# laoreja/HPLFlowNet

Hardware: AMD Instinct MI355X
Metric: point-pairs/sec + EPE3D, N=8192 FlyingThings3D, 1/2/4/8 MI355X (higher is better)
Workload: dtype f32 (wide layers: fp32 operands as scaled fp16 pairs, 3 partial products, fp32 accumulate); 1 GPU; full HPLFlowNet inference (7 levels, 19.3M params, random init), FT3D-like synthetic pair, N=8192, bs=1 per GPU; num_points=8192, step_includes_lattice_build=True, forward_streams=3, lattices_under_construction=3, exact_fallback_launches=0, lattice_launches_per_pair=34

## Files before the change

hplflownet_amd/bcl.py:

```python
import collections

import os

import torch
import torch.nn as nn

from . import _lib, ops
from .ops import ACT_LEAKY, ACT_NONE, LEAKY_RATE

__all__ = ['BilateralConvFlex', 'BilateralCorrelationFlex', 'sparse_sum', 'Conv1dReLU', 'Conv2dReLU',
           'Conv3dReLU', 'LEAKY_RATE']


class _ConvReLU(nn.Module):
    conv_cls = None

    def __init__(self, in_channels, out_channels, kernel_size=1, stride=1, padding=0, use_leaky=False,
                 bias=True):
        super(_ConvReLU, self).__init__()
        self.in_channels, self.out_channels, self.kernel_size = in_channels, out_channels, kernel_size
        self.use_leaky = use_leaky
        relu = nn.LeakyReLU(LEAKY_RATE, inplace=True) if use_leaky else nn.ReLU(inplace=True)
        self.composed_module = nn.Sequential(
            self.conv_cls(in_channels, out_channels, kernel_size=kernel_size, stride=stride, padding=padding,
# ... 215 lines not shown
        return ops.splat_raw(v, (csr_ptr, csr_pt, csr_w, norm), H, use_norm=False)

    @staticmethod
    def backward(ctx, grad_output):
        indices, = ctx.saved_tensors
        g = None
        if ctx.needs_input_grad[1]:
            g = grad_output[indices.reshape(-1).to(grad_output.device), :]
        return None, g, None, None


sparse_sum = SparseSum.apply


def _build_conv_stack(n_in, num_output, filter_size, last_relu, use_leaky, first_cls=Conv2dReLU,
                      plain_cls=nn.Conv2d):
    mods = []
    c = n_in
    for i, o in enumerate(num_output):
        ks = (filter_size, 1) if i == 0 else (1, 1)
        last = i == len(num_output) - 1
        if last and not last_relu:
            mods.append(plain_cls(c, o, kernel_size=ks))
        else:
            mods.append(first_cls(c, o, ks, use_leaky=use_leaky))
        c = o
    return nn.Sequential(*mods)


def _conv_of(m):
    return m.conv if isinstance(m, _ConvReLU) else m


def _run_conv_stack(x, stack, table, M, F, use_leaky, out=None, w0=None):
    n = len(stack)
    for i, m in enumerate(stack):
        conv = _conv_of(m)
        act = ACT_LEAKY if isinstance(m, _ConvReLU) else ACT_NONE
        o = out if i == n - 1 else None
        if i == 0:
            groups = table.groups() if conv.in_channels >= GROUPS_MIN_CHANNELS else None
            x = ops.gconv(x, conv.weight if w0 is None else w0, conv.bias, table.t, M, F, act=act,
                          bwd_mode=table.bwd_mode(x.shape[0]) if torch.is_grad_enabled() else 'scatter',
                          out=o, slope=_slope(use_leaky),
                          row_perm=table.perm if groups is None else None,
                          taps=table.taps if conv.in_channels >= 100 else None, tap_groups=groups,
                          reg_stride=getattr(table, 'reg_stride', 0),
                          tiles=(table.group_tiles() if groups is not None else table.perm_tiles) if table.t is not None else None)
        else:
            x = ops.gconv(x, conv.weight, conv.bias, None, M, 1, act=act, bwd_mode='dense', out=o,
                          slope=_slope(use_leaky))
    return x


class BilateralConvFlex(nn.Module):

    def __init__(self, d, neighborhood_size, num_input, num_output, DEVICE, use_bias, use_leaky, use_norm,
                 do_splat, do_slice, last_relu, chunk_size=1024 * 1024 * 25):
        super(BilateralConvFlex, self).__init__()
        self.d, self.d1 = d, d + 1
        self.neighborhood_size = neighborhood_size
        self.filter_size = (neighborhood_size + 1) ** self.d1 - neighborhood_size ** self.d1
        self.num_input, self.num_output = num_input, list(num_output)
        self.DEVICE = DEVICE
        self.use_bias, self.use_leaky, self.use_norm = use_bias, use_leaky, use_norm
        self.do_splat, self.do_slice, self.last_relu = do_splat, do_slice, last_relu
        self.MAX_SIZE = chunk_size
        self.register_buffer('feat_indices', torch.arange(num_input, dtype=torch.long))
        if do_slice:
            self.register_buffer('out_indices', torch.arange(num_output[-1], dtype=torch.long))
        self.blur_conv = _build_conv_stack(num_input, self.num_output, self.filter_size, last_relu, use_leaky)
        if do_slice and use_bias:
            self.register_parameter('bias', nn.Parameter(torch.zeros((num_output[-1],), dtype=torch.float32)))

    def get_filter_size(self):
        return self.filter_size

    def forward_cl(self, x, in_cloud, blur, out_cloud, out=None, keep=None, w0=None, folded=False):
        H = blur.t.shape[1]
        if self.do_splat:
            if in_cloud.H != H:
# ... 3 lines not shown
            else:
                s = ops.splat_raw(x, in_cloud.csr(), H, self.use_norm)
        else:
            if x.shape[0] != H:
                raise _lib.HplError('features have %d rows, blur table %d vertices' % (x.shape[0], H))
            s = x
        bias = (self.bias if self.use_bias else None) if self.do_slice else None
        mods = list(self.blur_conv)
        if folded:
            if torch.is_grad_enabled() or not self.do_slice or len(mods) < 2 or isinstance(mods[-1], _ConvReLU):
                raise _lib.HplError('the folded form is the inference forward of a slicing layer that ends in a bias-only 1x1')
            y = _run_conv_stack(s, mods[:-1], blur, H, self.filter_size, self.use_leaky, w0=w0)
            if keep is not None:
                keep.append(y)
            return ops.slice_raw(y, out_cloud.bary, out_cloud.off, out_cloud.N, out=out)
        if (self.do_slice and len(mods) >= 2 and not isinstance(mods[-1], _ConvReLU) and out_cloud.N < H):
            y = _run_conv_stack(s, mods[:-1], blur, H, self.filter_size, self.use_leaky)
            if keep is not None:
                keep.append(y)
            conv = mods[-1]
            b = conv.bias if bias is None else (conv.bias + bias if conv.bias is not None else bias)
            if torch.is_grad_enabled() and y.requires_grad:
                z = ops.SliceFn.apply(y, out_cloud, None)
            else:
                z = ops.slice_raw(y, out_cloud.bary, out_cloud.off, out_cloud.N)
            return ops.gconv(z, conv.weight, b, None, out_cloud.N, 1, act=ACT_NONE, bwd_mode='dense', out=out)
        if keep is not None and self.do_slice and len(mods) >= 2 and not isinstance(mods[-1], _ConvReLU):
            z = _run_conv_stack(s, mods[:-1], blur, H, self.filter_size, self.use_leaky)
            keep.append(z)
            conv = _conv_of(mods[-1])
            y = ops.gconv(z, conv.weight, conv.bias, None, H, 1, act=ACT_NONE, bwd_mode='dense', slope=_slope(self.use_leaky))
        else:
            y = _run_conv_stack(s, self.blur_conv, blur, H, self.filter_size, self.use_leaky,
                                out=None if self.do_slice else out)
            if keep is not None:
                keep.append(y)
        if not self.do_slice:
            return y
        if torch.is_grad_enabled() and (y.requires_grad or (bias is not None and bias.requires_grad)):
            z = ops.SliceFn.apply(y, out_cloud, bias)
            if out is not None:
                out.copy_(z)
                return out
            return z
        return ops.slice_raw(y, out_cloud.bary, out_cloud.off, out_cloud.N, bias=bias, out=out)

    def forward(self, features, in_barycentric, in_lattice_offset, blur_neighbors, out_barycentric,
                out_lattice_offset):
        if features.size(0) != 1:
            raise _lib.HplError('batch size must be 1 (reference README.md:57)')
        x = to_channel_last(features)
        H = blur_neighbors.size(-1)
        blur = nbr_table(blur_neighbors, x)
        in_cloud = cloud_tables(in_barycentric, in_lattice_offset, H, x) if self.do_splat else None
        out_cloud = cloud_tables(out_barycentric, out_lattice_offset, H, x) if self.do_slice else None
        return to_channel_first(self.forward_cl(x, in_cloud, blur, out_cloud))


class BilateralCorrelationFlex(nn.Module):

    def __init__(self, d, corr_filter_radius, corr_corr_radius, num_input, num_corr_output, num_output, DEVICE,
                 use_bias, use_leaky, use_norm, prev_corr_dim, last_relu, chunk_size=1024 * 1024 * 25):
        super(BilateralCorrelationFlex, self).__init__()
        self.d, self.d1 = d, d + 1
        self.corr_size = (corr_corr_radius + 1) ** self.d1 - corr_corr_radius ** self.d1
        self.filter_size = (corr_filter_radius + 1) ** self.d1 - corr_filter_radius ** self.d1
        self.num_input, self.prev_corr_dim = num_input, prev_corr_dim
# ... 68 lines not shown
```

hplflownet_amd/build.py:

```python
import os
import subprocess
import sys

HERE = os.path.dirname(os.path.abspath(__file__))
CSRC = os.path.join(HERE, 'csrc')
LIB = os.path.join(HERE, 'libhplbcl.so')
DIAG_LIB = os.path.join(HERE, 'libhplbcl_diag.so')
SOURCES = ['index_ops.hip', 'row_order.hip', 'splat_slice.hip', 'train_ops.hip', 'gconv.hip', 'gconv3.hip', 'wgrad3.hip', 'lattice.hip', 'lattice_fused.hip', 'executor.hip', 'lattice_builder.hip', 'lattice_query.hip', 'knn_interp.hip', 'rigid_fit.hip', 'motion_segment.hip', 'selfsup_loss.hip', 'ground_fit.hip', 'batch_io.hip', 'metrics.hip', 'transforms.hip']
FLAGS = ['--offload-arch=gfx950', '-O3', '-std=c++17', '-fPIC', '-munsafe-fp-atomics',
         '-ffp-contract=off',
         '-Wall', '-Wno-unused-function']


def needs_build():
    if not os.path.exists(LIB) or not os.path.exists(DIAG_LIB):
        return True
    t = os.path.getmtime(LIB)
    deps = [os.path.join(CSRC, f) for f in os.listdir(CSRC)] + \
           [os.path.join(os.path.dirname(HERE), 'include', 'hpl_bcl.h'), os.path.abspath(__file__)]
    return any(os.path.getmtime(d) > t for d in deps)


def build(force=False, verbose=False):
    if not force and not needs_build():
        return LIB
    hipcc = os.environ.get('HIPCC', '/opt/rocm/bin/hipcc')
    objs = []
    procs = []
    for src in SOURCES:
        path = os.path.join(CSRC, src)
        if not os.path.exists(path):
            continue
        obj = os.path.join(CSRC, src.replace('.hip', '.o'))
        cmd = [hipcc] + FLAGS + ['-c', path, '-o', obj]
        if verbose:
            print(' '.join(cmd))
        procs.append((src, subprocess.Popen(cmd, stdout=subprocess.PIPE, stderr=subprocess.STDOUT)))
        objs.append(obj)
    failed = False
    for src, p in procs:
        out, _ = p.communicate()
# ... 13 lines not shown
```

hplflownet_amd/csrc/gconv.hip:

```cpp
#include "common.h"
#include "gconv_common.h"
#include <cstdlib>
#include <cmath>
#include <string>

#include <stdlib.h>
#include <type_traits>

using namespace hpl;
using namespace hpl_gc;



namespace {

template <int BM, int BN, int WGM, int WGN, bool AVEC, int F_LDS, bool COMPACT = false>
__global__ void __launch_bounds__(64 * WGM * WGN, COMPACT ? 6 : 1) k_gconv(const GParams p) {
    constexpr int NT = 64 * WGM * WGN;
    constexpr int WTM = BM / WGM, WTN = BN / WGN;
    constexpr int TM = WTM / 32, TN = WTN / 32;
    constexpr int LDA_S = COMPACT ? BM + 1 : BM + 2;
    constexpr int LDB_S = BN;
    constexpr int A_ROWS_PER_PASS = NT / 8;
    constexpr int A_PASSES = BM / A_ROWS_PER_PASS;
// ... 582 lines not shown
    if (p.F == 1) {
        if (avec) k_gconv<BM, BN, WGM, WGN, true, 1><<<grid, 64 * WGM * WGN, 0, s>>>(p);
        else k_gconv<BM, BN, WGM, WGN, false, 1><<<grid, 64 * WGM * WGN, 0, s>>>(p);
    } else {
        if (avec) k_gconv<BM, BN, WGM, WGN, true, 15><<<grid, 64 * WGM * WGN, 0, s>>>(p);
        else k_gconv<BM, BN, WGM, WGN, false, 15><<<grid, 64 * WGM * WGN, 0, s>>>(p);
    }
}

}

namespace {
void launch_finish(const GParams &p, hipStream_t s) {
    const bool vec = p.N % 4 == 0 && p.ldy % 4 == 0 && aligned16(p.Y) && aligned16(p.partial) && (!p.bias || aligned16(p.bias)) &&
                     (!p.res || (p.ldres % 4 == 0 && aligned16(p.res))) && (!p.Y2 || (p.ldy2 % 4 == 0 && aligned16(p.Y2))) &&
                     p.M * p.N < (int64_t)0x7fffffff && p.res_mod < (int64_t)0x7fffffff;
    if (vec) {
        const int g = (int)imin(cdiv(p.M * (p.N / 4), 256), 2048);
        k_gconv_finish4<<<g, 256, 0, s>>>(p);
    } else {
        const int g = (int)imin(cdiv(p.M * p.N, 256), 2048);
        k_gconv_finish<<<g, 256, 0, s>>>(p);
    }
}
}

extern "C" int hpl_gconv_forward(const hpl_gconv_desc *d, hplStream stream) {
    GParams p;
    int rc = fill_params(d, p, "hpl_gconv_forward");
    if (rc != HPL_OK) return rc;
    if (p.M == 0) return HPL_OK;
    hipStream_t s = to_stream(stream);
    const bool avec = (p.C % 4 == 0) && (p.lda % 4 == 0) && aligned16(p.A);
    if (avec && p.Wt3 && launch_split3(p, s)) {
        if (p.splits > 1) launch_finish(p, s);
        HPL_CHECK_LAUNCH("hpl_gconv_forward");
        if (p.y_amax && !p.y_amax_done) return amax_launch(p.Y, p.ldy, p.M, p.N, p.y_amax, s, p.y_guard);
        return HPL_OK;
    }
    const int64_t t128 = cdiv(p.M, 128), t64 = cdiv(p.M, 64);
    const int nsel = p.N;
    if (nsel > 64) {
        const int64_t tn = cdiv(p.N, 128);
        if (t64 * tn >= 512) launch_cfg<64, 128, 2, 4>(p, avec, s);
        else launch_cfg<64, 64, 2, 2>(p, avec, s);
    } else if (nsel > 32) {
        launch_cfg<64, 64, 2, 2>(p, avec, s);
    } else {
        if (t128 >= 512) launch_cfg<128, 32, 4, 1>(p, avec, s);
        else launch_cfg<64, 32, 2, 1>(p, avec, s);
    }
    if (p.splits > 1) launch_finish(p, s);
    HPL_CHECK_LAUNCH("hpl_gconv_forward");
    if (p.y_amax) return amax_launch(p.Y, p.ldy, p.M, p.N, p.y_amax, s, p.y_guard);
    return HPL_OK;
}

namespace {
__global__ void __launch_bounds__(256) k_tile_index(const int32_t *__restrict__ nbr, int64_t stride, int F, int64_t M,
                                                    const int32_t *__restrict__ perm, int BM, int32_t *__restrict__ tile_idx,
                                                    int32_t *__restrict__ tile_mask) {
    __shared__ int masks[8];
    const int t = threadIdx.x;
    if (t < 8) masks[t] = 0;
    __syncthreads();
    const int64_t tile = blockIdx.x, m0 = tile * BM;
// ... 736 lines not shown
```

hplflownet_amd/csrc/gconv_common.h:

```cpp
#pragma once
#include "common.h"

namespace hpl_gc {

typedef float floatx16 __attribute__((ext_vector_type(16)));
typedef int int32x4_t __attribute__((ext_vector_type(4)));
typedef float float4_t __attribute__((ext_vector_type(4)));

__device__ float4_t buffer_load_f32x4(int32x4_t srsrc, int voffset, int soffset, int aux)
    __asm("llvm.amdgcn.raw.buffer.load.v4f32");


__device__ __forceinline__ int32x4_t make_rsrc(const void *base, int bytes) {
    union {
        int32x4_t v;
        struct { const void *p; int range; int cfg; } s;
    } u;
    u.s.p = base;
    u.s.range = bytes;
    u.s.cfg = 0x00020000;
    return u.v;
}

__host__ __device__ __forceinline__ float split_scale(float amax) {
// ... 94 lines not shown
        for (; x < 8; ++x) {
            int rows_x = 0;
            for (int r = 0; r * 8 < nchunks; ++r) {
                const int c = chunk_of(x, r);
                if (c < nchunks) rows_x += chunk_rows(c);
            }
            if (sq < rows_x) break;
            sq -= rows_x;
        }
        int row = 0;
        for (int r = 0;; ++r) {
            const int c = chunk_of(x, r);
            if (c >= nchunks) continue;
            const int n = chunk_rows(c);
            if (sq < n) { row = c * G + sq; break; }
            sq -= n;
        }
        tm = T - 1 - row;
        return;
    }
    constexpr int BAND = 8;
    const int band_sz = BAND * p.tiles_n;
    const int band = id / band_sz;
    const int in_band = id - band * band_sz;
    const int rows_in_band = min(BAND, p.tiles_m - band * BAND);
    tm = band * BAND + in_band % rows_in_band;
    tn = in_band / rows_in_band;
}
__device__ __forceinline__ void tile_coords(const GParams &p, int &tm, int &tn) { tile_coords(p, tm, tn, blockIdx.x); }


int fill_params(const hpl_gconv_desc *d, GParams &p, const char *who);
bool launch_split3(GParams &p, hipStream_t s);
bool split3_enabled();
int split_planes();
int amax_launch(const float *X, int64_t ld, int64_t rows, int cols, float *slot, hipStream_t s, unsigned *guard = nullptr);
constexpr int GUARD_GAP = 18;
__device__ __forceinline__ bool guard_tripped(const float *a_amax, const unsigned *a_guard) {
    if (!a_guard || !a_amax) return false;
    unsigned am;
    const float amf = a_amax[0];
    __builtin_memcpy(&am, &amf, 4);
    const unsigned g = a_guard[0];
    const unsigned rmin = g ? ~g : am;
    return (am >> 23) >= (rmin >> 23) + (unsigned)GUARD_GAP && (am >> 23) < 255u;
}
constexpr int RESID_SHIFT = 24;
inline bool split3_maybe(int64_t M, int C, int F, int N) {
    if (!(C >= 32 && N >= 256 && M >= 1024 && F <= 15)) return false;
    const int64_t tiles256 = ((M + 127) / 128) * ((N + 255) / 256);
    if (tiles256 >= 128) return true;
    if (F == 1) return M >= 8192;
    if (M >= 16384) return true;
    const int64_t nk = ((int64_t)F * C + BK - 1) / BK;
    const int64_t by_tiles = 256 / tiles256, by_k = nk / 16;
    return N % 256 == 0 && (by_tiles < by_k ? by_tiles : by_k) >= 2;
}

struct WParams {
    const float *A; int64_t lda; const int32_t *nbr; int64_t nbr_stride; int64_t reg_stride;
    int64_t M; int C; int F; int K;
    const float *dY; int64_t lddy; int N;
    float *dWt; int64_t ldw;
    int tiles_n; int64_t m_per_split;
    const int32_t *tap_m; const int32_t *tap_row; const int32_t *tap_ptr; int c_tiles;
    float *dbias;
// ... 7 lines not shown
```

hplflownet_amd/ops.py:

```python
import collections
import ctypes
import os

import torch

from . import _lib
from ._lib import GConvDesc, RelayoutJob, check, ptr, stream

ACT_NONE, ACT_LEAKY = 0, 1
LEAKY_RATE = 0.1


def _cl(x, what='activation'):
    if x.dim() != 2 or x.dtype != torch.float32 or not x.is_cuda or (x.shape[1] > 1 and x.stride(1) != 1):
        raise _lib.HplError('%s must be a channel-last 2-D float32 device tensor with unit channel stride, '
                            'got shape %s strides %s dtype %s device %s'
                            % (what, tuple(x.shape), x.stride(), x.dtype, x.device))
    return x


def _ld(x):
    return x.stride(0) if x.shape[0] > 1 else max(x.shape[1], x.stride(0))


# ... 1075 lines not shown
            self.total = prefix[-1]
            self.prefix_host = prefix
            raw = torch.frombuffer(bytearray(bytes(arr)), dtype=torch.uint8)
            self.dev_jobs = raw.to(dev)
            self.dev_prefix = torch.tensor(prefix, dtype=torch.int64, device=dev)
            self.buf = torch.empty(self.total, dtype=torch.float32, device=dev)
            self.dirty = False
        hi = len(self.jobs) if hi is None else hi
        if hi <= lo:
            return
        check(_lib.load().hpl_weight_relayout_batch(self.dev_jobs.data_ptr() + lo * ctypes.sizeof(RelayoutJob), hi - lo,
                                                    self.dev_prefix.data_ptr() + 8 * lo, self.prefix_host[hi] - self.prefix_host[lo],
                                                    ptr(self.buf), stream()), 'hpl_weight_relayout_batch')
        for job in list(self.jobs.values())[lo:hi]:
            job[4] = job[0]._version


BANK = None


def enable_weight_bank(on=True):
    global BANK
    BANK = WeightBank() if on else None
    return BANK


def _train_relayout(weight, R, Q, F, sr, sq, sf, base=0, mirror=False):
    if BANK is not None:
        return BANK.get(weight, R, Q, F, sr, sq, sf, base, mirror)
    fmap = _mirror_map(F, weight.device) if mirror else None
    return weight_relayout(weight, R, Q, F, sr, sq, sf, base=base, fmap=fmap)


MAX_TAPS_PER_PASS = 15


def gconv_passes(A, nbr, M, C, F, Wt, N, groups=None, bias=None, act=ACT_NONE, res=None, res_mod=0, out=None,
                 slope=LEAKY_RATE, row_perm=None, reg_stride=0, tiles=None, guard=True):
    regular = nbr is None and reg_stride > 0
    if not groups and (nbr is not None or regular) and F > MAX_TAPS_PER_PASS:
        groups = [(f0, min(F, f0 + MAX_TAPS_PER_PASS), None) for f0 in range(0, F, MAX_TAPS_PER_PASS)]
    W3 = split3_of(Wt) if (SPLIT3 and (nbr is not None or F == 1) and N >= SPLIT3_MIN_N and C >= SPLIT3_MIN_C) else None
    if not groups or not (nbr is not None or regular) or len(groups) < 2:
        return gconv_raw(A, nbr, M, C, F, Wt, N, bias=bias, act=act, res=res, res_mod=res_mod, out=out, slope=slope,
                         row_perm=row_perm, reg_stride=reg_stride, tiles=tiles if not isinstance(tiles, list) else None,
                         Wt3=W3, guard=guard)
    y = out
    gt = tiles if isinstance(tiles, list) and len(tiles) == len(groups) else [None] * len(groups)
    for i, (f0, f1, perm) in enumerate(groups):
        first, last = i == 0, i == len(groups) - 1
        w3 = W3.rows_from(f0 * C, Wt.shape[1]) if (W3 is not None and (f0 * C) % 8 == 0) else None
        y = gconv_raw(A[f0 * reg_stride:] if regular else A, None if regular else nbr[f0:f1], M, C, f1 - f0,
                      Wt[f0 * C:], N, bias=bias if first else None,
                      act=act if last else ACT_NONE, res=res if first else y, res_mod=res_mod if first else 0,
                      out=y, slope=slope, row_perm=perm, reg_stride=reg_stride, tiles=gt[i] if perm is not None else None,
                      Wt3=w3, guard=guard)
    return y


def _split3_entry(Wt, version):
    ev = torch.cuda.Event()
    w3 = weight_split3(Wt)
    ev.record()
    return [w3, version, ev, stream()]


def _split3_wait(entry):
    ev = entry[2]
    if ev is not None and stream() != entry[3]:
        if ev.query():
            entry[2] = None
        else:
            torch.cuda.current_stream().wait_event(ev)
    return entry[0]


def split3_of(Wt):
    job = getattr(Wt, '_hpl_bank_job', None)
    if job is not None:
        ent = job[5]
        if ent is None or ent[1] != job[4]:
            ent = job[5] = _split3_entry(Wt, job[4])
        return _split3_wait(ent)
    ent = getattr(Wt, '_hpl_split3', None)
    if ent is None or ent[1] != Wt._version:
        ent = Wt._hpl_split3 = _split3_entry(Wt, Wt._version)
    return _split3_wait(ent)


class GConvFn(torch.autograd.Function):

    @staticmethod
    def forward(ctx, A, weight, bias, nbr, M, c0, C, F, act, res, res_mod, bwd_mode, slope, row_perm=None,
                taps=None, groups=None, reg_stride=0, tiles=None):
        O = weight.shape[0]
        Ctot = weight.numel() // (O * F)
        Wt = _train_relayout(weight, C, O, F, F, Ctot * F, 1, base=c0 * F)
        Y = gconv_passes(A, nbr, M, C, F, Wt, O, groups, bias=bias, act=act, res=res, res_mod=res_mod, slope=slope,
                         row_perm=row_perm, reg_stride=reg_stride, tiles=tiles)
        ctx.reg_stride = reg_stride
        ctx.tiles = tiles
        ctx.groups = groups
        ctx.slope = slope
        ctx.row_perm = row_perm
        ctx.taps = taps
        ctx.save_for_backward(A, weight, nbr, Y if act != ACT_NONE else None)
        ctx.cfg = (M, c0, C, F, act, res is not None, res_mod, bwd_mode, bias is not None, Ctot)
        return Y

    @staticmethod
    def backward(ctx, g):
        A, weight, nbr, Y = ctx.saved_tensors
        M, c0, C, F, act, has_res, res_mod, bwd_mode, has_bias, Ctot = ctx.cfg
        O = weight.shape[0]
        g = g if (g.dim() == 2 and g.stride(1) == 1) else g.contiguous()
        if act == ACT_LEAKY:
            g = leaky_bwd(g, Y, ctx.slope)
        gA = gW = gb = gres = None
        if ctx.needs_input_grad[0]:
# ... 82 lines not shown
            dZ = gather_sum_raw(g, inv, K * Hv, F, O, 0).view(Hv, K * O)
            if ctx.needs_input_grad[0]:
                WzT = _train_relayout(weight, O, C, K, Ctot * K, K, 1, base=c0 * K)
                gf2 = gconv_raw(dZ, None, Hv, K * O, 1, WzT, C)
            if ctx.needs_input_grad[1]:
                dWz = wgrad_raw(f2, None, Hv, C, 1, dZ, K * O)
                gW = torch.zeros_like(weight)
                gW.view(O, Ctot, K)[:, c0:c0 + C, :] = dWz[:C, :K * O].view(C, K, O).permute(2, 0, 1)
        return gf2, gW, gb, gres, None, None, None, None, None, None, None


def corr_pc2(f2, weight, bias, res, table, H0, F, K, c0, C, slope):
    if torch.is_grad_enabled() and (f2.requires_grad or weight.requires_grad or (res is not None and res.requires_grad)):
        return CorrPc2Fn.apply(f2, weight, bias, res, table, H0, F, K, c0, C, slope)
    O = weight.shape[0]
    Ctot = weight.numel() // (O * K)
    key = (id(weight), c0, C, 'cols')
    hit = _WT_CACHE.get(key)
    if hit is None or hit[2] != weight._version or hit[1] is not weight or hit[3] != weight.data_ptr():
        img = _cols_image(weight, C, O, K, Ctot, c0)
        ev = torch.cuda.Event()
        ev.record()
        hit = _WT_CACHE[key] = [img, weight, weight._version, weight.data_ptr(), ev, stream()]
    elif hit[4] is not None and stream() != hit[5]:
        if hit[4].query():
            hit[4] = None
        else:
            torch.cuda.current_stream().wait_event(hit[4])
    Z = gconv_raw(f2, None, f2.shape[0], C, 1, hit[0], K * O)
    return gather_sum_raw(Z, table.t, F * H0, K, O, O, bias=bias, res=res, res_mod=H0, act=ACT_LEAKY, slope=slope)


def gconv(A, weight, bias, nbr, M, F, act=ACT_NONE, c0=0, C=None, res=None, res_mod=0, bwd_mode='scatter',
          out=None, slope=LEAKY_RATE, row_perm=None, taps=None, tap_groups=None, reg_stride=0, tiles=None):
    O = weight.shape[0]
    Ctot = weight.numel() // (O * F)
    C = Ctot if C is None else C
    if torch.is_grad_enabled() and (A.requires_grad or weight.requires_grad or
                                    (res is not None and res.requires_grad)):
        y = GConvFn.apply(A, weight, bias, nbr, M, c0, C, F, act, res, res_mod, bwd_mode, slope, row_perm,
                          taps() if callable(taps) else taps,
                          tap_groups() if callable(tap_groups) else tap_groups, reg_stride,
                          tiles() if callable(tiles) else tiles)
        if out is not None:
            out.copy_(y)
            return out
        return y
    Wt = _cached_relayout(weight, C, O, F, Ctot, c0)
    groups = tap_groups() if callable(tap_groups) else tap_groups
    return gconv_passes(A, nbr, M, C, F, Wt, O, groups, bias=bias, act=act, res=res, res_mod=res_mod, out=out,
                        slope=slope, row_perm=row_perm, reg_stride=reg_stride, tiles=tiles() if callable(tiles) else tiles)


_WT_CACHE = collections.OrderedDict()
_WT_CACHE_MAX = 512


def invalidate_weight_cache():
    global _WEIGHT_EPOCH
    _WT_CACHE.clear()
    _WEIGHT_EPOCH += 1


_WEIGHT_EPOCH = 0


def weight_epoch():
    return _WEIGHT_EPOCH


def _cached_relayout(weight, C, O, F, Ctot, c0):
    key = (id(weight), c0, C)
    hit = _WT_CACHE.get(key)
    if hit is not None and hit[2] == weight._version and hit[1] is weight and hit[3] == weight.data_ptr():
        ev = hit[4]
        if ev is not None:
            st = stream()
            if st != hit[5]:
                if ev.query():
                    hit[4] = None
                else:
                    torch.cuda.current_stream().wait_event(ev)
        return hit[0]
    Wt = weight_relayout(weight.detach(), C, O, F, F, Ctot * F, 1, base=c0 * F)
# ... 8 lines not shown
```

hplflownet_amd/plan.py:

```python
import ctypes
import os
import weakref

import time

import torch

from . import _lib, ops
from ._lib import Buf, LevelTables, Op, Ref, Weight, check, ptr, stream
from .bcl import GROUPS_MIN_CHANNELS, _ConvReLU, _conv_of, _slope
from .flownet import DeviceLattice, PairBlur

OP_GCONV, OP_SPLAT, OP_SLICE, OP_COPY, OP_LOAD = 1, 2, 3, 4, 5
OP_GSUM, OP_INVERT = 16, 17
F_NOYAMAX = 64
TBL_NONE, TBL_BLUR_PAIR, TBL_BLUR0, TBL_CORR1, TBL_CORR2, TBL_REGULAR, TBL_CSR_PAIR, TBL_CSR_C0, TBL_CLOUD0 = range(9)
ORD_NONE, ORD_PERM, ORD_GROUPS = 0, 1, 2
SYM_ZERO, SYM_N0, SYM_N1, SYM_NP, SYM_LEVEL0 = -1, 0, 1, 2, 8
S_H0, S_H1, S_HP, S_FH0, S_IN0, S_INP, S_FH1 = range(7)
BUF_OUT = -2

TAG_OTHER, TAG_WIDE_BLUR = 0, 1


# ... 349 lines not shown
                t.blur_perm_tidx, t.blur_perm_tmask = [x.data_ptr() for x in pb.perm_tiles]
        up = lv.blur[0]
        wide = hint[L] if isinstance(hint, (list, tuple)) else hint
        groups = up.groups() if wide else None
        if groups:
            t.n_up_groups = len(groups)
            tiles = up.group_tiles()
            for g, (f0, f1, pm) in enumerate(groups):
                t.up_group_cut[g], t.up_group_cut[g + 1] = f0, f1
                t.up_group_perm[g] = pm.data_ptr()
                if tiles is not None:
                    t.up_group_tidx[g], t.up_group_tmask[g] = tiles[g][0].data_ptr(), tiles[g][1].data_ptr()
                keep.append(pm)
        else:
            t.n_up_groups = 0
            pm = up.perm
            if pm is not None:
                t.up_perm = pm.data_ptr()
                if up.perm_tiles is not None:
                    t.up_perm_tidx, t.up_perm_tmask = [x.data_ptr() for x in up.perm_tiles]
        if lv.corr1 is not None:
            t.corr1, t.corr1_stride = lv.corr1.t.data_ptr(), lv.corr1.t.stride(0)
            pm = lv.corr1.perm
            if pm is not None:
                t.corr1_perm = pm.data_ptr()
                if lv.corr1.perm_tiles is not None:
                    t.corr1_perm_tidx, t.corr1_perm_tmask = [x.data_ptr() for x in lv.corr1.perm_tiles]
            t.corr2 = lv.corr2.t.data_ptr()
    lat._native_tables = (arr, n, keep)
    return lat._native_tables


class ForwardPlan(object):
    def __init__(self, model):
        self._model = weakref.ref(model)
        self.NLEV = model.NLEV
        self.epoch = ops.weight_epoch()
        self.bank = ops.WeightBank()
        self._images_ready = None
        self._images_stream = None
        with torch.no_grad():
            self.prog = self._program(model)
            self.bank.refresh()
        self._mark_images_written()
        self._sig = self._signature()
        L = _lib.load()
        P = self.prog
        ops_arr = (Op * len(P.ops))(*P.ops)
        bufs_arr = (Buf * len(P.bufs))(*[Buf(r, c) for r, c in P.bufs])
        w_arr = (Weight * len(P.weights))()
        wide = set(o.weight for o in P.ops if o.kind == OP_GCONV and o.table in (TBL_NONE, TBL_BLUR_PAIR, TBL_BLUR0, TBL_CORR1, TBL_CORR2)
                   and not (o.flags & 2) and o.N >= ops.SPLIT3_MIN_N and o.C >= ops.SPLIT3_MIN_C) if ops.SPLIT3 else set()
        self._split3 = {}
        done = {}
        for i, key in enumerate(P.weights):
            if key[0] == 'grad':
                w_arr[i].Wt, w_arr[i].rows, w_arr[i].ldw = self._grad_image(key[1])
                continue
            mirror = key[8] if len(key) > 8 else 0
            job = self.bank.jobs[self.bank._key(key[0], *key[1:8], mirror)]
            k_rows, ldw = job[6], job[7]
            w_arr[i].Wt = self.bank.buf.data_ptr() + 4 * job[2]
            w_arr[i].ldw, w_arr[i].rows = ldw, k_rows
            if i in wide and mirror != 2:
                if id(job) not in done:
                    img = self.bank.buf[job[2]:job[2] + k_rows * ldw].view(k_rows, ldw)
                    done[id(job)] = (img, ops.weight_split3(img))
                    self._split3[i] = done[id(job)]
                w3 = done[id(job)][1]
                w_arr[i].Wt3, w_arr[i].wt3_plane_stride, w_arr[i].wt3_planes = w3.planes.data_ptr(), w3.planes.stride(0), w3.P
                if w3.P == 2:
                    w_arr[i].w_amax = w3.amax.data_ptr()
        self._mark_images_written()
        b_arr = (ctypes.c_void_p * max(1, len(P.biases)))(*[(b if isinstance(b, int) else b.data_ptr()) for b in P.biases])
        self.handle = L.hpl_plan_create(ops_arr, len(P.ops), bufs_arr, len(P.bufs), w_arr, len(P.weights), b_arr,
                                        len(P.biases))
        if not self.handle:
            raise _lib.HplError('hpl_plan_create failed: %s' % L.hpl_last_error().decode())
        self._lib = L
        self.hint = model.lattice_hint()
        self._ws = {}
        self._slot = 0
        self.slots = 4
        self._fence = {}

    def _program(self, model):
        P = build_program(model, self.bank, fold=model.fold_up())
        for f in P.folds:
            f.ensure()
        return P

    def __del__(self):
        try:
            if getattr(self, 'handle', None):
                self._lib.hpl_plan_destroy(self.handle)
            self._ws.clear()
        except Exception:
            pass

    @property
# ... 150 lines not shown
```

hplflownet_amd/train_plan.py:

```python
import ctypes

import numpy as np
import torch

from . import _lib, ops
from ._lib import LevelTables, RelayoutJob, check, ptr, stream
from .bcl import _ConvReLU
from .plan import (BUF_OUT, ForwardPlan, ORD_NONE, OP_GCONV, OP_GSUM, OP_INVERT, S_FH0, S_FH1, S_H0, S_H1, S_HP, S_IN0, S_INP, SYM_N0, SYM_N1,
                   SYM_NP, SYM_LEVEL0, SYM_ZERO, TBL_BLUR0, TBL_BLUR_PAIR, TBL_CORR1, TBL_CORR2, TBL_CSR_C0, TBL_CSR_PAIR, TBL_NONE,
                   TBL_REGULAR, _R, build_program, level_tables, lsym)

OP_WGRAD, OP_LEAKY_BWD, OP_COLSUM, OP_SPLAT_BWD, OP_PSUM, OP_REGROUP, OP_ZERO, OP_EPE3D, OP_VCOPY, OP_UNLAYOUT = range(6, 16)
OP_SPLAT, OP_COPY = 2, 4
F_ACCUM, F_SCATTER, F_TAPS, F_SIDE, F_INVERSE, F_NOGUARD = 1, 2, 4, 8, 16, 32


class _Sim(object):

    def __init__(self, P, nlev):
        self.P = P
        sym = {SYM_ZERO: 0, SYM_N0: 3, SYM_N1: 4, SYM_NP: 7}
        n0, n1 = 3, 4
        for L in range(nlev):
            h0, h1 = 5 + 2 * L, 6 + 2 * L
# ... 217 lines not shown

    def _slice(self, m):
        P, cond = self.P, m['cond']
        g = self.G(m['out'])
        assert self.sim.written(g, cond)
        ga = self.G(m['a']).columns(0, m['C'])
        P.splat(g, ga, m['level'], TBL_CSR_C0, lsym(m['level'], S_H0), m['C'], False, flags=F_ACCUM if self.sim.claim(ga, cond) else 0)
        P.meta[-1] = None
        if m['bias'] >= 0:
            b = P.biases[m['bias']]
            P.raw(OP_COLSUM, a=g, M=m['N'], C=m['C'], bias=self._gvec(b), flags=F_SIDE)
            self._stores(b)


def check_batch_step(pc1, pc2, sf, lat):
    if getattr(lat, 'ragged', False):
        raise _lib.HplError('ragged batches are for inference: a training batch holds pairs of equal point counts')
    if any(getattr(x, 'dim', lambda: 0)() != 3 for x in (pc1, pc2, sf)) or pc1.shape[1] != 3 or pc2.shape[1] != 3:
        raise _lib.HplError('a training batch is (B, 3, N) clouds and flow, got %s / %s / %s'
                            % tuple(tuple(getattr(x, 'shape', ())) for x in (pc1, pc2, sf)))
    B = int(pc1.shape[0])
    if int(pc2.shape[0]) != B or tuple(sf.shape) != tuple(pc1.shape):
        raise _lib.HplError('training batch: pc1 %s, pc2 %s and sf %s do not pair up' % (tuple(pc1.shape), tuple(pc2.shape), tuple(sf.shape)))
    if not 1 <= B <= 64:
        raise _lib.HplError('a training batch holds 1 .. 64 pairs, got %d' % B)
    lb = int(getattr(lat, 'batch', 1) or 1)
    if lb != B:
        raise _lib.HplError('training batch of %d pairs, but the lattice was built for %d' % (B, lb))
    return B


class TrainPlan(ForwardPlan):

    def __init__(self, model, reducer=None, side_stream=True):
        self.params = [p for p in model.parameters()]
        if any(not p.requires_grad for p in self.params):
            raise _lib.HplError('the native training step expects every parameter to require a gradient')
        from . import parallel
        self.reducer = reducer if reducer is not None else parallel.GradAllReducer(self.params, overlap=False)
        dev = self.params[0].device
        order = [p for b in self.reducer.buckets for p in b]
        assert len(order) == len(self.params)
        self.gflat = torch.zeros(sum((p.numel() + 3) // 4 * 4 for p in order), dtype=torch.float32, device=dev)
        self._goff, self._bucket_of, o = {}, {}, 0
        self.bucket_range = []
        for bi, b in enumerate(self.reducer.buckets):
            o0 = o
            for p in b:
                self._goff[id(p)] = o
                self._bucket_of[id(p)] = bi
                p.grad = self.gflat[o:o + p.numel()].view(p.shape)
                o += (p.numel() + 3) // 4 * 4
            self.bucket_range.append((o0, o))
        self.reducer.adopt_flat(self.gflat, self.bucket_range)
        self.pflat = torch.zeros_like(self.gflat)
        with torch.no_grad():
            for p in order:
                o = self._goff[id(p)]
                v = self.pflat[o:o + p.numel()].view(p.shape)
                v.copy_(p.data)
                p.data = v
        ops.invalidate_weight_cache()
        torch.cuda.current_stream(dev).synchronize()
        self._adam = None
        self.loss = torch.zeros(1, dtype=torch.float32, device=dev)
        if isinstance(side_stream, torch.cuda.Stream):
# ... 316 lines not shown
```

Measured before the change: 501.7 point-pairs/s.

## Add narrow-output three-plane bf16 MFMA gconv kernel for 15-tap blur layers

Adds a new HIP kernel, gconv3n, for gathered lattice convolutions with 15 taps and narrow outputs (33 to 64 channels). Each fp32 operand is split into three bf16 planes and combined with six 32x32x16 MFMA products per K slice. A/B staging is double-buffered through LDS, and the K loop skips slices whose taps have no neighbors in the tile. The forward plan now precomputes three-plane weight splits for eligible splat-only blur layers and passes a narrow3 flag down the Python path. The kernel is gated by an environment variable that defaults to off, and the training plan disables it; the extra Wt3 pointers may still change which existing split3 path is chosen.

Result: slower. 490.6 point-pairs/s (-2.2%).

```diff
diff --git a/hplflownet_amd/bcl.py b/hplflownet_amd/bcl.py
--- a/hplflownet_amd/bcl.py
+++ b/hplflownet_amd/bcl.py
@@ -271,7 +271,7 @@
     return m.conv if isinstance(m, _ConvReLU) else m
 
 
-def _run_conv_stack(x, stack, table, M, F, use_leaky, out=None, w0=None):
+def _run_conv_stack(x, stack, table, M, F, use_leaky, out=None, w0=None, narrow3=False):
     n = len(stack)
     for i, m in enumerate(stack):
         conv = _conv_of(m)
@@ -285,7 +285,8 @@
                           row_perm=table.perm if groups is None else None,
                           taps=table.taps if conv.in_channels >= 100 else None, tap_groups=groups,
                           reg_stride=getattr(table, 'reg_stride', 0),
-                          tiles=(table.group_tiles() if groups is not None else table.perm_tiles) if table.t is not None else None)
+                          tiles=(table.group_tiles() if groups is not None else table.perm_tiles) if table.t is not None else None,
+                          narrow3=narrow3)
         else:
             x = ops.gconv(x, conv.weight, conv.bias, None, M, 1, act=act, bwd_mode='dense', out=o,
                           slope=_slope(use_leaky))
@@ -355,7 +356,7 @@
             y = ops.gconv(z, conv.weight, conv.bias, None, H, 1, act=ACT_NONE, bwd_mode='dense', slope=_slope(self.use_leaky))
         else:
             y = _run_conv_stack(s, self.blur_conv, blur, H, self.filter_size, self.use_leaky,
-                                out=None if self.do_slice else out)
+                                out=None if self.do_slice else out, narrow3=self.do_splat and not self.do_slice)
             if keep is not None:
                 keep.append(y)
         if not self.do_slice:
diff --git a/hplflownet_amd/build.py b/hplflownet_amd/build.py
--- a/hplflownet_amd/build.py
+++ b/hplflownet_amd/build.py
@@ -6,7 +6,7 @@
 CSRC = os.path.join(HERE, 'csrc')
 LIB = os.path.join(HERE, 'libhplbcl.so')
 DIAG_LIB = os.path.join(HERE, 'libhplbcl_diag.so')
-SOURCES = ['index_ops.hip', 'row_order.hip', 'splat_slice.hip', 'train_ops.hip', 'gconv.hip', 'gconv3.hip', 'wgrad3.hip', 'lattice.hip', 'lattice_fused.hip', 'executor.hip', 'lattice_builder.hip', 'lattice_query.hip', 'knn_interp.hip', 'rigid_fit.hip', 'motion_segment.hip', 'selfsup_loss.hip', 'ground_fit.hip', 'batch_io.hip', 'metrics.hip', 'transforms.hip']
+SOURCES = ['index_ops.hip', 'row_order.hip', 'splat_slice.hip', 'train_ops.hip', 'gconv.hip', 'gconv3.hip', 'gconv3n.hip', 'wgrad3.hip', 'lattice.hip', 'lattice_fused.hip', 'executor.hip', 'lattice_builder.hip', 'lattice_query.hip', 'knn_interp.hip', 'rigid_fit.hip', 'motion_segment.hip', 'selfsup_loss.hip', 'ground_fit.hip', 'batch_io.hip', 'metrics.hip', 'transforms.hip']
 FLAGS = ['--offload-arch=gfx950', '-O3', '-std=c++17', '-fPIC', '-munsafe-fp-atomics',
          '-ffp-contract=off',
          '-Wall', '-Wno-unused-function']
diff --git a/hplflownet_amd/csrc/gconv.hip b/hplflownet_amd/csrc/gconv.hip
--- a/hplflownet_amd/csrc/gconv.hip
+++ b/hplflownet_amd/csrc/gconv.hip
@@ -638,6 +638,11 @@
     if (p.M == 0) return HPL_OK;
     hipStream_t s = to_stream(stream);
     const bool avec = (p.C % 4 == 0) && (p.lda % 4 == 0) && aligned16(p.A);
+    if (avec && p.Wt3 && launch_narrow3(p, s)) {
+        HPL_CHECK_LAUNCH("hpl_gconv_forward");
+        if (p.y_amax) return amax_launch(p.Y, p.ldy, p.M, p.N, p.y_amax, s, p.y_guard);
+        return HPL_OK;
+    }
     if (avec && p.Wt3 && launch_split3(p, s)) {
         if (p.splits > 1) launch_finish(p, s);
         HPL_CHECK_LAUNCH("hpl_gconv_forward");
diff --git a/hplflownet_amd/csrc/gconv3n.hip b/hplflownet_amd/csrc/gconv3n.hip
--- /dev/null
+++ b/hplflownet_amd/csrc/gconv3n.hip
@@ -0,0 +1,302 @@
+#include "common.h"
+#include "gconv_common.h"
+
+#include <stdlib.h>
+#include <type_traits>
+
+using namespace hpl;
+using namespace hpl_gc;
+
+typedef __bf16 bf16x8 __attribute__((ext_vector_type(8)));
+typedef __bf16 bf16x2 __attribute__((ext_vector_type(2)));
+typedef float float2_t __attribute__((ext_vector_type(2)));
+typedef unsigned u32x4 __attribute__((ext_vector_type(4)));
+typedef unsigned u32x2 __attribute__((ext_vector_type(2)));
+
+namespace {
+
+__device__ __forceinline__ void split2(float x0, float x1, unsigned &h, unsigned &m, unsigned &l) {
+    const float2_t v = {x0, x1};
+    h = __builtin_bit_cast(unsigned, __builtin_convertvector(v, bf16x2));
+    const float r0 = x0 - __builtin_bit_cast(float, h << 16), r1 = x1 - __builtin_bit_cast(float, h & 0xffff0000u);
+    const float2_t rv = {r0, r1};
+    m = __builtin_bit_cast(unsigned, __builtin_convertvector(rv, bf16x2));
+    const float s0 = r0 - __builtin_bit_cast(float, m << 16), s1 = r1 - __builtin_bit_cast(float, m & 0xffff0000u);
+    const float2_t sv = {s0, s1};
+    l = __builtin_bit_cast(unsigned, __builtin_convertvector(sv, bf16x2));
+}
+
+constexpr int NBM = 64, NBN = 64, NNT = 256, NF = 15;
+constexpr int A_PLANE = 2 * NBM * 16;
+constexpr int A_STAGE = 3 * A_PLANE;
+constexpr int B_PLANE = 4 * NBN * 16;
+constexpr int B_STAGE = 3 * B_PLANE;
+constexpr int B_BASE = 2 * A_STAGE;
+constexpr int IS_BASE = B_BASE + 2 * B_STAGE;
+constexpr int KLIST = 64;
+constexpr int SMEM_BYTES = IS_BASE + NF * NBM * 4 + 8 * 4 + KLIST * 2;
+static_assert(SMEM_BYTES <= 40960, "four workgroups per CU");
+
+__global__ void __launch_bounds__(NNT, 4) k_gconv3n(const GParams p) {
+    __shared__ __attribute__((aligned(16))) unsigned char smem[SMEM_BYTES];
+    int *Is = reinterpret_cast<int *>(smem + IS_BASE);
+    int *masks = Is + NF * NBM;
+    unsigned short *Ks = reinterpret_cast<unsigned short *>(masks + 8);
+
+    const int t = threadIdx.x, lane = t & 63;
+    const int wave = __builtin_amdgcn_readfirstlane(t >> 6);
+    const int wm = wave >> 1, wn = wave & 1;
+    const int li = lane & 31, hi = lane >> 5;
+
+    const int j = (int)blockIdx.x;
+    const int tile_m = p.row_perm ? (p.tile_idx ? p.tile_mask[(int64_t)j * 8 + 6] : p.tiles_m - 1 - j) : j;
+    const int64_t m0 = (int64_t)tile_m * NBM;
+    const int64_t m_out = m0 + wm * 32 + li;
+    const int my_v = m_out < p.M ? (p.row_perm ? p.row_perm[m_out] : (int)m_out) : -1;
+
+    const int lda_b = (int)(p.lda * 4);
+    if (p.tile_idx) {
+        const int32_t *ti = p.tile_idx + (int64_t)tile_m * NF * NBM;
+        if (t < 8) masks[t] = p.tile_mask[(int64_t)tile_m * 8 + t];
+        for (int i = t; i < NF * NBM; i += NNT) {
+            const int row = ti[i];
+            Is[i] = row >= 0 ? row * lda_b : (int)0x80000000;
+        }
+    } else {
+        if (t < 8) masks[t] = 0;
+        __syncthreads();
+        const int r = t & (NBM - 1);
+        const int64_t m = m0 + r;
+        const int v = m < p.M ? (p.row_perm ? p.row_perm[m] : (int)m) : -1;
+        int mybits = 0;
+        for (int f = t >> 6; f < NF; f += NNT / NBM) {
+            const int row = v >= 0 ? p.nbr[(int64_t)f * p.nbr_stride + v] : -1;
+            Is[f * NBM + r] = row >= 0 ? row * lda_b : (int)0x80000000;
+            mybits |= (row >= 0) ? (1 << f) : 0;
+        }
+        if (mybits) {
+            atomicOr(masks, mybits);
+            atomicOr(masks + 2 + (r >> 5), mybits);
+        }
+    }
+    __syncthreads();
+    const int tapmask = __builtin_amdgcn_readfirstlane(masks[0]) & 0x7fff;
+    const int bmask = __builtin_amdgcn_readfirstlane(masks[2 + wm]);
+    const int nk = (p.K + BK - 1) / BK;
+    int nsl, ks_reg;
+    {
+        bool need = false;
+        int e = 0;
+        if (lane < nk) {
+            const int f_lo = (lane * BK) / p.C;
+            const int f_hi = min((lane * BK + BK - 1) / p.C, NF - 1);
+            need = (tapmask & ((1 << f_lo) | (1 << f_hi))) != 0;
+            e = lane | (f_lo << 10) | (f_hi > f_lo ? (1 << 14) : 0);
+        }
+        const unsigned long long bal = __ballot(need);
+        if (need) Ks[__popcll(bal & ((1ull << lane) - 1ull))] = (unsigned short)e;
+        nsl = __popcll(bal);
+        ks_reg = (int)Ks[lane];
+    }
+    auto ks_at = [&](int sl) { return __builtin_amdgcn_readlane(ks_reg, sl); };
+
+    constexpr unsigned OOB = 0x80000000u;
+    const int32x4_t rsrc_a = make_rsrc(p.A, (int)p.a_bytes);
+    const int k4 = t & 3, arow = t >> 2;
+    const unsigned w3_bytes = (unsigned)(p.w_bytes / 2);
+    __amdgpu_buffer_rsrc_t rsrc_b[3];
+#pragma unroll
+    for (int pl = 0; pl < 3; ++pl)
+        rsrc_b[pl] = __builtin_amdgcn_make_buffer_rsrc(
+            const_cast<unsigned char *>(reinterpret_cast<const unsigned char *>(p.Wt3) + (int64_t)pl * p.w3_plane_stride),
+            (short)0, (int)w3_bytes, 0x00020000);
+    const unsigned ldw16 = (unsigned)p.ldw * 16u;
+    const unsigned b_colofs = ((unsigned)lane < (unsigned)p.ldw) ? (unsigned)lane * 16u : OOB;
+
+    float4_t ra[2][2];
+    auto load_a = [&](auto set_tag, int e) {
+        constexpr int SET = decltype(set_tag)::value;
+        const int32x4_t rs = rsrc_a;
+        const int f0 = (e >> 10) & 15;
+        const int cb = (e & 1023) * BK - f0 * p.C + k4 * 4;
+        unsigned o[2];
+#pragma unroll
+        for (int i = 0; i < 2; ++i) {
+            int c = cb + i * 16, f = f0;
+            const bool wrap = c >= p.C;
+            c = wrap ? c - p.C : c;
+            f += wrap ? 1 : 0;
+            const unsigned row = (unsigned)Is[min(f, NF - 1) * NBM + arow];
+            o[i] = (f < NF ? row : OOB) + (unsigned)c * 4u;
+        }
+#pragma unroll
+        for (int i = 0; i < 2; ++i) {
+            float4_t &dst = ra[SET][i];
+            asm volatile("buffer_load_dwordx4 %0, %1, %2, 0 offen" : "=v"(dst) : "v"(o[i]), "s"(rs) : "memory");
+        }
+    };
+    auto pin = [&](auto set_tag) {
+        constexpr int SET = decltype(set_tag)::value;
+#pragma unroll
+        for (int i = 0; i < 2; ++i) {
+            float4_t &x = ra[SET][i];
+            asm volatile("" : "+v"(x));
+        }
+    };
+    const int kb_w = k4 >> 1;
+    unsigned char *const a_wr = smem + (kb_w * NBM + (arow ^ (kb_w << 3))) * 16 + (k4 & 1) * 8;
+    auto store_a = [&](auto set_tag, int h) {
+        constexpr int SET = decltype(set_tag)::value;
+        const float4_t v = h ? ra[SET][1] : ra[SET][0];
+        unsigned char *base = a_wr + h * A_STAGE;
+        unsigned h0, m0_, l0, h1, m1, l1;
+        split2(v.x, v.y, h0, m0_, l0);
+        split2(v.z, v.w, h1, m1, l1);
+        *reinterpret_cast<u32x2 *>(base) = u32x2{h0, h1};
+        *reinterpret_cast<u32x2 *>(base + A_PLANE) = u32x2{m0_, m1};
+        *reinterpret_cast<u32x2 *>(base + 2 * A_PLANE) = u32x2{l0, l1};
+    };
+    auto load_b = [&](int kt, int st) {
+        const unsigned off = (unsigned)(kt * (BK / 8) + wave) * ldw16 + b_colofs;
+#pragma unroll
+        for (int pl = 0; pl < 3; ++pl)
+            __builtin_amdgcn_raw_ptr_buffer_load_lds(
+                rsrc_b[pl], (__attribute__((address_space(3))) void *)(smem + B_BASE + st * B_STAGE + pl * B_PLANE + wave * NBN * 16),
+                16, (int)off, 0, 0, 0);
+    };
+
+    floatx16 acc;
+#pragma unroll
+    for (int r = 0; r < 16; ++r) acc[r] = 0.f;
+    const unsigned a_rofs = (unsigned)((hi * NBM + ((wm * 32 + li) ^ (hi << 3))) * 16);
+    const unsigned b_rofs = (unsigned)(B_BASE + (hi * NBN + wn * 32 + li) * 16);
+
+    auto compute = [&](int h, int sb, bool need) {
+        if (!need) return;
+        constexpr int PA[6] = {0, 0, 1, 0, 2, 1};
+        constexpr int PB[6] = {0, 1, 0, 2, 0, 1};
+        u32x4 af[3], bf[3];
+#pragma unroll
+        for (int pl = 0; pl < 3; ++pl) {
+            af[pl] = *reinterpret_cast<const u32x4 *>(smem + h * A_STAGE + pl * A_PLANE + a_rofs);
+            bf[pl] = *reinterpret_cast<const u32x4 *>(smem + sb * B_STAGE + pl * B_PLANE + h * 2 * NBN * 16 + b_rofs);
+        }
+#pragma unroll
+        for (int q = 0; q < 6; ++q)
+            acc = __builtin_amdgcn_mfma_f32_32x32x16_bf16(__builtin_bit_cast(bf16x8, bf[PB[q]]), __builtin_bit_cast(bf16x8, af[PA[q]]), acc, 0, 0, 0);
+    };
+    auto wait_lgkm0 = []() { __builtin_amdgcn_s_waitcnt((63 & 0xF) | ((63 >> 4) << 14) | (0x7 << 4) | (0x0 << 8)); };
+    auto wait_all = []() { __builtin_amdgcn_s_waitcnt(0x7 << 4); };
+
+    using S0 = std::integral_constant<int, 0>;
+    using S1 = std::integral_constant<int, 1>;
+    if (nsl > 0) {
+        load_b(ks_at(0) & 1023, 0);
+        load_a(S0{}, ks_at(0));
+        if (nsl > 1) load_a(S1{}, ks_at(1));
+        wait_all();
+        pin(S0{}); pin(S1{});
+        store_a(S0{}, 0);
+        wait_lgkm0();
+        asm volatile("s_barrier" ::: "memory");
+        auto slice = [&](int sl, auto set_tag, auto other_tag) {
+            const int sb = decltype(set_tag)::value;
+            const int e = ks_at(sl);
+            const int f_lo = (e >> 10) & 15;
+            const bool need = ((bmask >> f_lo) | (((e >> 14) & 1) ? (bmask >> (f_lo + 1)) : 0)) & 1;
+            compute(0, sb, need);
+            store_a(set_tag, 1);
+            if (sl + 1 < nsl) load_b(ks_at(sl + 1) & 1023, sb ^ 1);
+            if (sl + 2 < nsl) load_a(set_tag, ks_at(sl + 2));
+            wait_lgkm0();
+            asm volatile("s_barrier" ::: "memory");
+            compute(1, sb, need);
+            if (sl + 1 < nsl) store_a(other_tag, 0);
+            wait_all();
+            pin(set_tag);
+            asm volatile("s_barrier" ::: "memory");
+        };
+        for (int sl = 0; sl < nsl; sl += 2) {
+            slice(sl, S0{}, S1{});
+            if (sl + 1 < nsl) slice(sl + 1, S1{}, S0{});
+        }
+    }
+
+    const __amdgpu_buffer_rsrc_t rs_y = __builtin_amdgcn_make_buffer_rsrc((void *)p.Y, (short)0, 0x7fffffff, 0x00020000);
+    const int32x4_t rs_r = make_rsrc(p.res ? (const void *)p.res : (const void *)p.Y, p.res ? 0x7fffffff : 0);
+    const __amdgpu_buffer_rsrc_t rs_y2 = __builtin_amdgcn_make_buffer_rsrc(
+        p.Y2 ? (void *)p.Y2 : (void *)p.Y, (short)0, p.Y2 ? 0x7fffffff : 0, 0x00020000);
+    const bool has_res = p.res != nullptr, has_y2 = p.Y2 != nullptr;
+    const int m = my_v;
+    int rr = m;
+    if (has_res && p.res_mod < p.M) {
+        const int q = (int)((float)rr * (1.0f / (float)p.res_mod));
+        rr -= (int)__umul24((unsigned)q, (unsigned)p.res_mod);
+        rr = rr < 0 ? rr + (int)p.res_mod : (rr >= (int)p.res_mod ? rr - (int)p.res_mod : rr);
+    }
+    const unsigned yrow = __umul24((unsigned)m, (unsigned)p.ldy * 4u), rrow = __umul24((unsigned)rr, (unsigned)p.ldres * 4u);
+    const unsigned y2row = __umul24((unsigned)m, (unsigned)p.ldy2 * 4u);
+    auto at = [&](bool row_ok, unsigned row_b, int n) { return (row_ok && n < p.N) ? row_b + (unsigned)n * 4u : OOB; };
+    auto col_of = [&](int q) { return wn * 32 + 8 * q + 4 * hi; };
+    const int32x4_t rs_b = make_rsrc(p.bias ? (const void *)p.bias : (const void *)p.Y, p.bias ? p.N * 4 : 0);
+    float4_t rv[4], bv[4];
+#pragma unroll
+    for (int q = 0; q < 4; ++q) bv[q] = buffer_load_f32x4(rs_b, col_of(q) * 4, 0, 0);
+    if (has_res) {
+#pragma unroll
+        for (int q = 0; q < 4; ++q) rv[q] = buffer_load_f32x4(rs_r, (int)at(m >= 0, rrow, col_of(q)), 0, 0);
+    }
+#pragma unroll
+    for (int q = 0; q < 4; ++q) {
+        const int n = col_of(q);
+        const float bb[4] = {bv[q].x, bv[q].y, bv[q].z, bv[q].w};
+        const float rr4[4] = {rv[q].x, rv[q].y, rv[q].z, rv[q].w};
+        unsigned ob[4];
+#pragma unroll
+        for (int c = 0; c < 4; ++c) {
+            float x = acc[4 * q + c] + bb[c];
+            if (has_res) x += rr4[c];
+            if (p.act == HPL_ACT_LEAKY) x = x > 0.f ? x : p.slope * x;
+            ob[c] = __builtin_bit_cast(unsigned, x);
+        }
+        const u32x4 o = {ob[0], ob[1], ob[2], ob[3]};
+        __builtin_amdgcn_raw_buffer_store_b128(o, rs_y, (int)at(m >= 0, yrow, n), 0, 0);
+        if (has_y2) __builtin_amdgcn_raw_buffer_store_b128(o, rs_y2, (int)at(m >= 0 && m < (int)p.rows2, y2row, n), 0, 0);
+    }
+}
+
+}
+
+constexpr bool NARROW3_DEFAULT = false;
+static bool narrow3_enabled() {
+    static const bool on = [] {
+        const char *e = getenv("HPL_NARROW3");
+        if (!e || !e[0]) return NARROW3_DEFAULT;
+        return !(e[0] == '0' && e[1] == 0);
+    }();
+    return on;
+}
+
+bool hpl_gc::launch_narrow3(GParams &p, hipStream_t s) {
+    constexpr int64_t min_rows = 16384;
+    if (!narrow3_enabled() || !split3_enabled() || !p.Wt3 || p.planes != 3) return false;
+    if (p.F != NF || !p.nbr || p.scat || p.M < min_rows) return false;
+    if (p.C < 32 || p.C % 4 != 0 || p.K > KLIST * BK || p.N <= 32 || p.N > NBN || p.N % 4 != 0) return false;
+    if (p.lda % 4 != 0 || !aligned16(p.A) || !aligned16(p.Wt3) || p.w3_plane_stride % 16 != 0) return false;
+    if ((p.w_bytes / (p.ldw * 4)) % 8 != 0 || p.w_bytes / (p.ldw * 4) < p.K) return false;
+    const int64_t lim = (int64_t)0x7fffffff;
+    const bool epi = p.M < (1 << 24) && p.M * p.ldy * 4 < lim && p.ldy * 4 < (1 << 24) &&
+                     (!p.res || (p.res_mod > 0 && p.res_mod < (1 << 24) && imin(p.res_mod, p.M) * p.ldres * 4 < lim && p.ldres * 4 < (1 << 24))) &&
+                     (!p.Y2 || (p.rows2 * p.ldy2 * 4 < lim && p.ldy2 * 4 < (1 << 24))) &&
+                     p.ldy % 4 == 0 && aligned16(p.Y) && (!p.bias || aligned16(p.bias)) &&
+                     (!p.res || (p.ldres % 4 == 0 && aligned16(p.res))) && (!p.Y2 || (p.ldy2 % 4 == 0 && aligned16(p.Y2)));
+    if (!epi) return false;
+    p.tiles_m = (int)cdiv(p.M, NBM);
+    p.tiles_n = 1;
+    p.splits = 1; p.partial = nullptr;
+    if (p.tile_bm != NBM) p.tile_idx = nullptr;
+    p.epi_fast = 1;
+    p.y_amax_done = 0;
+    k_gconv3n<<<p.tiles_m, NNT, 0, s>>>(p);
+    return true;
+}
diff --git a/hplflownet_amd/csrc/gconv_common.h b/hplflownet_amd/csrc/gconv_common.h
--- a/hplflownet_amd/csrc/gconv_common.h
+++ b/hplflownet_amd/csrc/gconv_common.h
@@ -150,6 +150,7 @@
 
 int fill_params(const hpl_gconv_desc *d, GParams &p, const char *who);
 bool launch_split3(GParams &p, hipStream_t s);
+bool launch_narrow3(GParams &p, hipStream_t s);
 bool split3_enabled();
 int split_planes();
 int amax_launch(const float *X, int64_t ld, int64_t rows, int cols, float *slot, hipStream_t s, unsigned *guard = nullptr);
diff --git a/hplflownet_amd/ops.py b/hplflownet_amd/ops.py
--- a/hplflownet_amd/ops.py
+++ b/hplflownet_amd/ops.py
@@ -1131,15 +1131,21 @@
     return weight_relayout(weight, R, Q, F, sr, sq, sf, base=base, fmap=fmap)
 
 
+def narrow3_shape(C, F, N):
+    return F == 15 and C >= 32 and C % 4 == 0 and F * C <= 2048 and 32 < N <= 64 and N % 4 == 0
+
+
 MAX_TAPS_PER_PASS = 15
 
 
 def gconv_passes(A, nbr, M, C, F, Wt, N, groups=None, bias=None, act=ACT_NONE, res=None, res_mod=0, out=None,
-                 slope=LEAKY_RATE, row_perm=None, reg_stride=0, tiles=None, guard=True):
+                 slope=LEAKY_RATE, row_perm=None, reg_stride=0, tiles=None, guard=True, narrow3=False):
     regular = nbr is None and reg_stride > 0
     if not groups and (nbr is not None or regular) and F > MAX_TAPS_PER_PASS:
         groups = [(f0, min(F, f0 + MAX_TAPS_PER_PASS), None) for f0 in range(0, F, MAX_TAPS_PER_PASS)]
     W3 = split3_of(Wt) if (SPLIT3 and (nbr is not None or F == 1) and N >= SPLIT3_MIN_N and C >= SPLIT3_MIN_C) else None
+    if W3 is None and narrow3 and SPLIT3 and nbr is not None and not groups and narrow3_shape(C, F, N):
+        W3 = split3_of(Wt, planes=3)
     if not groups or not (nbr is not None or regular) or len(groups) < 2:
         return gconv_raw(A, nbr, M, C, F, Wt, N, bias=bias, act=act, res=res, res_mod=res_mod, out=out, slope=slope,
                          row_perm=row_perm, reg_stride=reg_stride, tiles=tiles if not isinstance(tiles, list) else None,
@@ -1157,9 +1163,9 @@
     return y
 
 
-def _split3_entry(Wt, version):
+def _split3_entry(Wt, version, planes=None):
     ev = torch.cuda.Event()
-    w3 = weight_split3(Wt)
+    w3 = weight_split3(Wt, planes=planes)
     ev.record()
     return [w3, version, ev, stream()]
 
@@ -1174,16 +1180,16 @@
     return entry[0]
 
 
-def split3_of(Wt):
+def split3_of(Wt, planes=None):
     job = getattr(Wt, '_hpl_bank_job', None)
     if job is not None:
         ent = job[5]
         if ent is None or ent[1] != job[4]:
-            ent = job[5] = _split3_entry(Wt, job[4])
+            ent = job[5] = _split3_entry(Wt, job[4], planes)
         return _split3_wait(ent)
     ent = getattr(Wt, '_hpl_split3', None)
     if ent is None or ent[1] != Wt._version:
-        ent = Wt._hpl_split3 = _split3_entry(Wt, Wt._version)
+        ent = Wt._hpl_split3 = _split3_entry(Wt, Wt._version, planes)
     return _split3_wait(ent)
 
 
@@ -1332,7 +1338,7 @@
 
 
 def gconv(A, weight, bias, nbr, M, F, act=ACT_NONE, c0=0, C=None, res=None, res_mod=0, bwd_mode='scatter',
-          out=None, slope=LEAKY_RATE, row_perm=None, taps=None, tap_groups=None, reg_stride=0, tiles=None):
+          out=None, slope=LEAKY_RATE, row_perm=None, taps=None, tap_groups=None, reg_stride=0, tiles=None, narrow3=False):
     O = weight.shape[0]
     Ctot = weight.numel() // (O * F)
     C = Ctot if C is None else C
@@ -1349,7 +1355,8 @@
     Wt = _cached_relayout(weight, C, O, F, Ctot, c0)
     groups = tap_groups() if callable(tap_groups) else tap_groups
     return gconv_passes(A, nbr, M, C, F, Wt, O, groups, bias=bias, act=act, res=res, res_mod=res_mod, out=out,
-                        slope=slope, row_perm=row_perm, reg_stride=reg_stride, tiles=tiles() if callable(tiles) else tiles)
+                        slope=slope, row_perm=row_perm, reg_stride=reg_stride, tiles=tiles() if callable(tiles) else tiles,
+                        narrow3=narrow3)
 
 
 _WT_CACHE = collections.OrderedDict()
diff --git a/hplflownet_amd/plan.py b/hplflownet_amd/plan.py
--- a/hplflownet_amd/plan.py
+++ b/hplflownet_amd/plan.py
@@ -405,6 +405,8 @@
 
 
 class ForwardPlan(object):
+    narrow3 = True
+
     def __init__(self, model):
         self._model = weakref.ref(model)
         self.NLEV = model.NLEV
@@ -424,6 +426,8 @@
         w_arr = (Weight * len(P.weights))()
         wide = set(o.weight for o in P.ops if o.kind == OP_GCONV and o.table in (TBL_NONE, TBL_BLUR_PAIR, TBL_BLUR0, TBL_CORR1, TBL_CORR2)
                    and not (o.flags & 2) and o.N >= ops.SPLIT3_MIN_N and o.C >= ops.SPLIT3_MIN_C) if ops.SPLIT3 else set()
+        narrow = set(o.weight for o in P.ops if o.kind == OP_GCONV and o.table == TBL_BLUR_PAIR and not (o.flags & 2)
+                     and ops.narrow3_shape(o.C, o.F, o.N)) if (ops.SPLIT3 and self.narrow3) else set()
         self._split3 = {}
         done = {}
         for i, key in enumerate(P.weights):
@@ -435,10 +439,10 @@
             k_rows, ldw = job[6], job[7]
             w_arr[i].Wt = self.bank.buf.data_ptr() + 4 * job[2]
             w_arr[i].ldw, w_arr[i].rows = ldw, k_rows
-            if i in wide and mirror != 2:
+            if (i in wide or i in narrow) and mirror != 2:
                 if id(job) not in done:
                     img = self.bank.buf[job[2]:job[2] + k_rows * ldw].view(k_rows, ldw)
-                    done[id(job)] = (img, ops.weight_split3(img))
+                    done[id(job)] = (img, ops.weight_split3(img, planes=None if i in wide else 3))
                     self._split3[i] = done[id(job)]
                 w3 = done[id(job)][1]
                 w_arr[i].Wt3, w_arr[i].wt3_plane_stride, w_arr[i].wt3_planes = w3.planes.data_ptr(), w3.planes.stride(0), w3.P
diff --git a/hplflownet_amd/train_plan.py b/hplflownet_amd/train_plan.py
--- a/hplflownet_amd/train_plan.py
+++ b/hplflownet_amd/train_plan.py
@@ -273,6 +273,8 @@
 
 class TrainPlan(ForwardPlan):
 
+    narrow3 = False
+
     def __init__(self, model, reducer=None, side_stream=True):
         self.params = [p for p in model.parameters()]
         if any(not p.requires_grad for p in self.params):
```
